# lyclyc52/Segment-Anything-NeRF

Measured on AMD Instinct MI355X. Metric: rays/sec (RGB+256-d SAM feat) at 512×512, 1/2/4/8 MI355X; PSNR vs ref, higher is better.
Workload: dtype fp32-equivalent: fp32 in the reference's op order for everything that decides a discrete result (near/far, bins, proposal grids + MLPs, compositing, sample_pdf); grid_mlp (32->64->64->16 per sample), the SAM head (163->256x5) and the mask head (143->256->256->K per sample) as f16x3: each fp32 produc

## Files before the change

segment-anything-nerf_amd/csrc/raymarch.hip:

```cpp
#include <algorithm>
#include <cmath>
#include <cstdlib>
#include <cstring>
#include <type_traits>

#include "f16x3.h"
#include "raymarch_device.h"
#include "samnerf_common.h"
#include "sh_device.h"
#include "wave_box.h"

using namespace samnerf;

namespace samnerf {
int sam_head_forward(const samnerf_model* m, const float* rows, uint32_t N, float* samvit,
                     float* packed, hipStream_t s, uint32_t ld = 256u, bool pack = true);
size_t sam_head_packed_floats();
int mask_head_forward(const samnerf_model* m, const GridDesc<16>& grid, const float* u_f, const float* w_f,
                      const float* geo_f, uint32_t N, float* out, RayTiles tiles, float* packed,
                      hipStream_t s);
size_t mask_head_packed_floats();
size_t mask_train_workspace_bytes(uint32_t N);
size_t mask_train_workspace_bytes(int mask_kind, uint32_t N);
int mask_train_forward(const samnerf_model* m, const GridDesc<16>& grid, const float* u_f, const float* w_f,
// ... 1491 lines not shown
}

struct SgridArgs {
    uint32_t N;
    RayTiles tiles;
    GridDesc<16> grid;
    const float* u_in;
    const float* w_in;
    float* rows;
    uint32_t* rows_tap;
    uint32_t tap_stride;
    unsigned long long* paths;
};


template <int T, int MODE>
__global__ void __launch_bounds__(256) k_sgrid(SgridArgs a) {
    constexpr int TQ = T / 4;
    __shared__ float part[3][8][64];
    const uint32_t lane = threadIdx.x & 63u, q = threadIdx.x >> 6;
    const uint32_t r = xcd_chunk(blockIdx.x, (a.N + 63u) / 64u) * 64u + lane;
    const uint32_t level = blockIdx.y;
    const bool live = r < a.N;
    const uint32_t N = a.N, rr = live ? r : N - 1;
    const LevelDesc lv = a.grid.lv[level];
    float acc[8];
#pragma unroll
    for (int c = 0; c < 8; ++c) acc[c] = 0.0f;
    const int k0 = (int)q * TQ;
    float ux = a.u_in[((size_t)k0 * 3 + 0) * N + rr];
    float uy = a.u_in[((size_t)k0 * 3 + 1) * N + rr];
    float uz = a.u_in[((size_t)k0 * 3 + 2) * N + rr];
    float w = a.w_in[(size_t)k0 * N + rr];
    for (int k = k0; k < k0 + TQ; ++k) {
        const int kn = k + 1 < k0 + TQ ? k + 1 : k;
        const float nx = a.u_in[((size_t)kn * 3 + 0) * N + rr];
        const float ny = a.u_in[((size_t)kn * 3 + 1) * N + rr];
        const float nz = a.u_in[((size_t)kn * 3 + 2) * N + rr];
        const float nw = a.w_in[(size_t)kn * N + rr];
        float f[8];
        if (__builtin_amdgcn_ballot_w64(w != 0.0f) == 0) {
        } else if constexpr (MODE == kLookRef) {
            lookup_level3_ref<8>(a.grid.emb, lv, ux, uy, uz, f);
#pragma unroll
            for (int c = 0; c < 8; ++c) acc[c] = acc[c] + w * f[c];
        } else {
            lookup_level3<8>(a.grid.emb, lv, ux, uy, uz, f);
            const f2v wv = {w, w};
#pragma unroll
            for (int c = 0; c < 8; c += 2) {
                const f2v s = f2v{acc[c], acc[c + 1]} + wv * f2v{f[c], f[c + 1]};
                acc[c] = s.x;
                acc[c + 1] = s.y;
            }
        }
        ux = nx;
        uy = ny;
        uz = nz;
        w = nw;
    }
    if (q > 0) {
#pragma unroll
        for (int c = 0; c < 8; ++c) part[q - 1][c][lane] = acc[c];
    }
    __syncthreads();
    if (q > 0 || !live) return;
#pragma unroll
    for (int c = 0; c < 8; ++c) acc[c] = ((acc[c] + part[0][c][lane]) + part[1][c][lane]) + part[2][c][lane];
    float4* dst = reinterpret_cast<float4*>(a.rows + (size_t)a.tiles(r) * kRow + level * 8u);
    dst[0] = make_float4(acc[0], acc[1], acc[2], acc[3]);
    dst[1] = make_float4(acc[4], acc[5], acc[6], acc[7]);
}

constexpr uint32_t kBoxSlots = 256;

#ifndef SAMNERF_DIAG_SGRID_WAVES
#define SAMNERF_DIAG_SGRID_WAVES 4
#endif
#ifndef SAMNERF_SGRID_UNI
#define SAMNERF_SGRID_UNI 1
#endif
constexpr bool SGRID_UNI = SAMNERF_SGRID_UNI;

template <int T, bool TAP = false>
__global__ void __launch_bounds__(256)
#if SAMNERF_DIAG_SGRID_WAVES
__attribute__((amdgpu_waves_per_eu(SAMNERF_DIAG_SGRID_WAVES, SAMNERF_DIAG_SGRID_WAVES)))
#endif
k_sgrid_box4(SgridArgs a) {
    constexpr int TQ = T / 4;
    __shared__ float4 smem[4][kBoxSlots * 2];
    const uint32_t lane = threadIdx.x & 63u, q = threadIdx.x >> 6;
    const uint32_t r = xcd_chunk(blockIdx.x, (a.N + 63u) / 64u) * 64u + lane;
    const uint32_t g = blockIdx.y;
    const bool live = r < a.N;
    const uint32_t N = a.N, rr = live ? r : N - 1;
    const LevelDesc L[4] = {a.grid.lv[4 * g], a.grid.lv[4 * g + 1], a.grid.lv[4 * g + 2],
                            a.grid.lv[4 * g + 3]};
    const uint32_t li = lane & 3u;
    const LevelDesc mine = {li == 0 ? L[0].off : li == 1 ? L[1].off : li == 2 ? L[2].off : L[3].off,
                            li == 0 ? L[0].size : li == 1 ? L[1].size : li == 2 ? L[2].size : L[3].size,
                            li == 0 ? L[0].res : li == 1 ? L[1].res : li == 2 ? L[2].res : L[3].res,
                            0u,
                            li == 0 ? L[0].fres : li == 1 ? L[1].fres : li == 2 ? L[2].fres : L[3].fres,
                            li == 0 ? L[0].ftop : li == 1 ? L[1].ftop : li == 2 ? L[2].ftop : L[3].ftop};
    float* slice = reinterpret_cast<float*>(smem[q]);
    const char* base = reinterpret_cast<const char*>(a.grid.emb);
    float acc[4][8];
#pragma unroll
    for (int l = 0; l < 4; ++l)
#pragma unroll
        for (int c = 0; c < 8; ++c) acc[l][c] = 0.0f;
    const int k0 = (int)q * TQ;
    const char* ub = reinterpret_cast<const char*>(a.u_in);
    const char* wb = reinterpret_cast<const char*>(a.w_in);
    const uint32_t N4 = N * 4u;
    auto ld = [](const char* b, uint32_t off) { return *reinterpret_cast<const float*>(b + off); };
    float ux = ld(ub, ((uint32_t)k0 * 3u + 0u) * N4 + rr * 4u);
    float uy = ld(ub, ((uint32_t)k0 * 3u + 1u) * N4 + rr * 4u);
    float uz = ld(ub, ((uint32_t)k0 * 3u + 2u) * N4 + rr * 4u);
    float w = ld(wb, (uint32_t)k0 * N4 + rr * 4u);
    for (int k = k0; k < k0 + TQ; ++k) {
        const uint32_t kn = (uint32_t)(k + 1 < k0 + TQ ? k + 1 : k);
        const float nx = ld(ub, (kn * 3u + 0u) * N4 + rr * 4u);
        const float ny = ld(ub, (kn * 3u + 1u) * N4 + rr * 4u);
        const float nz = ld(ub, (kn * 3u + 2u) * N4 + rr * 4u);
        const float nw = ld(wb, kn * N4 + rr * 4u);
#ifdef SAMNERF_DIAG_VARIANTS
        if (a.paths && lane == 0u && __builtin_amdgcn_ballot_w64(w != 0.0f) == 0) atomicAdd(a.paths + 3, 1ull);
#endif
        if (__builtin_amdgcn_ballot_w64(w != 0.0f) != 0) {
            const f2v wv = {w, w};
            auto add = [&](int l, const float* f) {
#pragma unroll
                for (int c = 0; c < 8; c += 2) {
                    const f2v s2 = f2v{acc[l][c], acc[l][c + 1]} + wv * f2v{f[c], f[c + 1]};
                    acc[l][c] = s2.x;
                    acc[l][c + 1] = s2.y;
                }
            };
            const URange ur = wave_urange(ux, uy, uz);
            const bool ordered = wave_positions_ordered(ux, uy, uz);
            uint32_t p0, p1, p2;
            pbox_lane(mine, ur, p0, p1, p2);
#pragma unroll
            for (int l = 0; l < 4; ++l) {
                const PBox b = pbox_read(p0, p1, p2, l);
                float f[8];
                uint32_t* rt = nullptr;
                if (TAP && live && r % a.tap_stride == 0u)
                    rt = a.rows_tap + ((size_t)(r / a.tap_stride) * T + k) * 128u + (4 * g + l) * 8;
#ifdef SAMNERF_DIAG_VARIANTS
                if (a.paths && lane == 0u) {
                    const int path = (SGRID_UNI && b.uni && ordered) ? 0 : b.slots <= kBoxSlots ? 1 : 2;
                    atomicAdd(a.paths + path, 1ull);
                    if (path == 1) {
                        atomicAdd(a.paths + 4, (unsigned long long)b.slots);
                        atomicAdd(a.paths + 5, (unsigned long long)(b.ex * b.ey * b.ez));
                    }
                }
#endif
                if (SGRID_UNI && b.uni && ordered) {
                    const uint32_t dx = b.ex - 1u, dy = b.ey - 1u, dz = b.ez - 1u;
                    uint32_t rows[8];
#pragma unroll
                    for (int c = 0; c < 8; ++c)
                        rows[c] = dense_or_hash_row(b.x0 + (c & 1) * dx, b.y0 + ((c >> 1) & 1) * dy,
                                                    b.z0 + (c >> 2) * dz, L[l]);
                    if (rt) {
#pragma unroll
                        for (int c = 0; c < 8; ++c) rt[c] = rows[c];
                    }
                    lookup_level3_uniform<8>(a.grid.emb, L[l], rows, ux, uy, uz, f);
                } else if (b.slots <= kBoxSlots) {
                    wave_lds_sync();
                    stage_pbox<8>(base, L[l], b, slice, lane);
                    wave_lds_sync();
                    if (ordered)
                        lookup_level3_pbox<8, false>(a.grid.emb, L[l], b, slice, ux, uy, uz, f, rt);
                    else
                        lookup_level3_pbox<8, true>(a.grid.emb, L[l], b, slice, ux, uy, uz, f, rt);
                } else {
                    if (rt) tap_direct_rows<8>(L[l], ux, uy, uz, rt);
                    lookup_level3<8>(a.grid.emb, L[l], ux, uy, uz, f);
                }
                add(l, f);
            }
        }
        ux = nx;
        uy = ny;
        uz = nz;
        w = nw;
    }
    __syncthreads();
    float* part = reinterpret_cast<float*>(smem);
    if (q > 0) {
#pragma unroll
        for (int l = 0; l < 4; ++l)
#pragma unroll
            for (int c = 0; c < 8; ++c) part[((q - 1) * 32 + l * 8 + c) * 64 + lane] = acc[l][c];
    }
    __syncthreads();
    if (q > 0 || !live) return;
    float* dst = a.rows + (size_t)a.tiles(r) * kRow + g * 32u;
#pragma unroll
    for (int l = 0; l < 4; ++l) {
        float v[8];
#pragma unroll
        for (int c = 0; c < 8; ++c) {
            const int i = l * 8 + c;
            v[c] = ((acc[l][c] + part[(0 * 32 + i) * 64 + lane]) + part[(1 * 32 + i) * 64 + lane]) +
                   part[(2 * 32 + i) * 64 + lane];
        }
        reinterpret_cast<float4*>(dst + l * 8)[0] = make_float4(v[0], v[1], v[2], v[3]);
        reinterpret_cast<float4*>(dst + l * 8)[1] = make_float4(v[4], v[5], v[6], v[7]);
    }
}

constexpr uint32_t kBwdBoxCells = 64;

struct DetAcc {
    unsigned long long* acc;
    const uint32_t* hdr;
    int log2n;
};

__device__ __forceinline__ bool sgrid_det_nonfinite(const DetAcc& d) { return d.hdr[1] != 0u; }

__device__ __forceinline__ int sgrid_det_shift(const DetAcc& d) {
    int e = 0;
    frexpf(__uint_as_float(d.hdr[0]), &e);
    return 61 - d.log2n - e;
}

template <int T, bool DET = false>
__global__ void __launch_bounds__(256)
k_sgrid_backward(uint32_t N, RayTiles tiles, GridDesc<16> g, const float* __restrict__ u_in,
                 const float* __restrict__ w_in, const float* __restrict__ grad, uint32_t gstride,
                 float* __restrict__ gemb, uint32_t max_cells, uint32_t run_res, DetAcc det = {}) {
    __shared__ float box[4][kBwdBoxCells * 8];
    __shared__ uint32_t list[4][kBwdBoxCells];
    const uint64_t t = (uint64_t)blockIdx.x * blockDim.x + threadIdx.x;
    const uint32_t r = (uint32_t)(t >> 3), ch = (uint32_t)(t & 7u), lane = threadIdx.x & 63u;
    const uint32_t wv = threadIdx.x >> 6;
    const uint32_t level = blockIdx.y;
    if (((t & ~(uint64_t)63) >> 3) >= N) return;
#ifdef SG_DIAG_MINLEVEL
    if (level < SG_DIAG_MINLEVEL) return;
#endif
    const bool live = r < N;
    const uint32_t rr = live ? r : N - 1;
    const LevelDesc d = g.lv[level];
    const float gv = live ? grad[(size_t)tiles(rr) * gstride + level * 8u + ch] : 0.0f;
    float* base = gemb + (size_t)d.off * 8u + ch;
    float* slice = box[wv];
    uint32_t* rows = list[wv];
    const uint32_t top = d.res - 1u;
    const int k0 = (int)(blockIdx.z * T / gridDim.z), k1 = (int)((blockIdx.z + 1) * T / gridDim.z);
    const bool run = !DET && max_cells == 0u && d.res <= run_res;
    const bool fixed = DET && !sgrid_det_nonfinite(det);
    const double dscale = fixed ? ldexp(1.0, sgrid_det_shift(det)) : 0.0;
    unsigned long long* const dbase = fixed ? det.acc + (size_t)d.off * 8u + ch : nullptr;
    uint32_t prow[8];
    float pval[8];
#pragma unroll
    for (int c = 0; c < 8; ++c) {
        prow[c] = 0xFFFFFFFFu;
        pval[c] = 0.0f;
    }
    for (int k = k0; k < k1; ++k) {
        const float ux = u_in[((size_t)k * 3 + 0) * N + rr];
        const float uy = u_in[((size_t)k * 3 + 1) * N + rr];
        const float uz = u_in[((size_t)k * 3 + 2) * N + rr];
        const float wk = w_in[(size_t)k * N + rr];
        if (__builtin_amdgcn_ballot_w64(wk != 0.0f) == 0) continue;
        const float wg = wk * gv;
        uint32_t cx, cy, cz;
        float fx, fy, fz;
        locate_axis(ux, d, cx, fx);
        locate_axis(uy, d, cy, fy);
        locate_axis(uz, d, cz, fz);
        const uint32_t nx = min(cx + 1u, top), ny = min(cy + 1u, top), nz = min(cz + 1u, top);
        const uint32_t x0 = (uint32_t)wave_imin((int)cx), x1 = (uint32_t)wave_imax((int)nx);
        const uint32_t y0 = (uint32_t)wave_imin((int)cy), y1 = (uint32_t)wave_imax((int)ny);
        const uint32_t z0 = (uint32_t)wave_imin((int)cz), z1 = (uint32_t)wave_imax((int)nz);
        const uint32_t ex = x1 - x0 + 1u, ey = y1 - y0 + 1u, ez = z1 - z0 + 1u;
        const uint32_t cells = ex * ey * ez;
        if (!DET && cells <= max_cells) {
            reinterpret_cast<float4*>(slice + lane * 8u)[0] = make_float4(0.0f, 0.0f, 0.0f, 0.0f);
            reinterpret_cast<float4*>(slice + lane * 8u)[1] = make_float4(0.0f, 0.0f, 0.0f, 0.0f);
            wave_lds_sync();
            const uint32_t X[2] = {cx - x0, nx - x0};
            const uint32_t Y[2] = {(cy - y0) * ex, (ny - y0) * ex};
            const uint32_t Z[2] = {(cz - z0) * ex * ey, (nz - z0) * ex * ey};
#pragma unroll
            for (int c = 0; c < 8; ++c) {
                const float wx = (c & 1) ? fx : 1.0f - fx;
                const float wy = (c & 2) ? fy : 1.0f - fy;
// ... 178 lines not shown
    z[r * 3] = a;
    z[r * 3 + 1] = b;
    z[r * 3 + 2] = c;
}

__global__ void __launch_bounds__(256)
k_sample_pdf(const float* __restrict__ bins, const float* __restrict__ weights, uint32_t N,
             uint32_t T0, uint32_t T, Lin u, float* __restrict__ out, int32_t* __restrict__ inds) {
    const uint32_t r = blockIdx.x * blockDim.x + threadIdx.x;
    if (r >= N) return;
    const float* w = weights + (size_t)r * T0;
    const float* b = bins + (size_t)r * (T0 + 1);
    const float wsum = torch_row_sum((int)T0, [&](int i) { return w[i] + 0.01f; });
    sample_pdf_walk(
        (int)T0, (int)T, u, wsum, [&](int i) { return w[i]; },
        [&](int i) { return b[i]; },
        [&](int j, float v, int ind) {
            out[(size_t)r * T + j] = v;
            if (inds) inds[(size_t)r * T + j] = ind;
        });
}

__global__ void __launch_bounds__(256)
k_composite(const float* __restrict__ rb, const float* __restrict__ sig, uint32_t N, uint32_t T,
            float* __restrict__ w) {
    const uint32_t r = blockIdx.x * blockDim.x + threadIdx.x;
    if (r >= N) return;
    double cum = 0.0;
    for (uint32_t k = 0; k < T; ++k) {
        const float ds = (rb[(size_t)r * (T + 1) + k + 1] - rb[(size_t)r * (T + 1) + k]) *
                         sig[(size_t)r * T + k];
        w[(size_t)r * T + k] = composite_step(ds, cum, k == T - 1);
    }
}

}



namespace {

struct Workspace {
    float* snf;
    float4* rec;
    float* bins1;
    float* bins2;
    float* wtmp;
    float* u_f;
    float* w_f;
    float* rows;
    float* packed;
    uint4* gpack;
    int* gexp;
    float* geo_f;
    float* mpacked;
    float* aeff;
    float* mlog;
    float* xsum;
    uint32_t* n1_list;
    uint32_t* n1_cnt;
    uint64_t* n1_mask;
    uint32_t* n1_base;
    double* n1_std;
    float* n1_stf;
    size_t bytes;
};

size_t align256(size_t b) { return (b + 255) & ~(size_t)255; }

int lookup_mode() {
    const char* v = diag_env("SAMNERF_LOOKUP");
    if (!v || !*v) return kLookAuto;
    if (!strcmp(v, "ref")) return kLookRef;
    if (!strcmp(v, "box")) return kLookBox4;
    if (!strcmp(v, "box4")) return kLookBox4;
    return kLookPacked;
}

thread_local hipEvent_t g_stage_events[8];
thread_local uint32_t g_n_stage_events = 0;
thread_local samnerf_taps g_taps = {};
thread_local uint32_t g_taps_n = 0;
thread_local bool g_taps_on = false;
thread_local uint32_t g_last_forms[4] = {};

void mark_stage(uint32_t i, hipStream_t s) {
    if (i < g_n_stage_events && g_stage_events[i]) (void)hipEventRecord(g_stage_events[i], s);
}

constexpr uint32_t kBox4MinRays = 32768;

uint32_t final_classes() {
    const char* v = diag_env("SAMNERF_FINAL_CLASSES");
    return (v && atoi(v) == 0) ? 0u : 1u;
}

int final_layout(const FinalArgs& fa) {
    const char* v = diag_env("SAMNERF_FINAL_LAY");
    if (v && atoi(v) == 0) return 0;
    for (int kb = 0; kb < 2; ++kb)
        if (fa.kdense[kb] != kLay1Dense[kb] || fa.khashed[kb] != kLay1Hashed[kb]) return 0;
    if (fa.hbit == 0u) return 0;
    return fa.gs.inv_b2 != 0.0f ? 1 : 0;
}

void set_hash_slots(FinalArgs& fa, const GridDesc<16>& g) {
    fa.hbit = fa.hm8 = 0u;
    uint32_t S = 0u;
    for (int kb = 0; kb < 2; ++kb)
        for (int q = 0; q < 4; ++q) {
            fa.hoff8[kb][q] = 0u;
            if (!((fa.khashed[kb] >> q) & 1u)) continue;
            const LevelDesc& a = g.lv[final_level(kb, 0, q)];
            const LevelDesc& b = g.lv[final_level(kb, 1, q)];
            if (!S) S = a.size;
            if (a.size != S || b.size != S || (S & (S - 1u)) || b.off != a.off + S || a.res > S || b.res > S ||
                (uint64_t)S * 8u > (1ull << 31))
                return;
            fa.hoff8[kb][q] = a.off * 8u;
        }
    if (!S) return;
    fa.hbit = S * 8u;
    fa.hm8 = (S - 1u) * 8u;
}

bool pack_weights(const samnerf_model* m) {
#ifdef SAMNERF_DIAG_VARIANTS
    return true;
#else
    return m->reuse_packed == 0;
#endif
}

bool box4_ok(const GridDesc<16>& g) {
    for (int l = 0; l < 16; ++l)
        if (g.lv[l].res > 1023u) return false;
    return true;
}

template <int T, bool FIRST>
void launch_prop_sigma(int look, uint32_t N, hipStream_t s, const PropArgs& pa) {
    const uint32_t nb = prop_sigma_blocks<T>(N);
    uint32_t kd = 0, kh = 0;
    for (int l = 0; l < 5; ++l) {
        kd |= (pa.grid.lv[l].flags & kHashed) ? 0u : 1u << l;
        kh |= (pa.grid.lv[l].flags & kHashed) ? 1u << l : 0u;
    }
    const char* pl = diag_env("SAMNERF_PROP_LAY");
    bool small_res = true;
    for (int l = 0; l < 5; ++l)
        if ((pa.grid.lv[l].flags & kHashed) && pa.grid.lv[l].res > pa.grid.lv[l].size) small_res = false;
    const bool lay = (look == kLookPacked || look == kLookAuto) && pa.gs.inv_b2 != 0.0f &&
                     !(pl && atoi(pl) == 0) && small_res && pa.rec;
    const bool lay_ok = lay && ((kd == 0x07u && kh == 0x18u) || (kd == 0x03u && kh == 0x1Cu));
    g_last_forms[T == 128 ? 0 : 1] = lay_ok ? kd | kh << 8 : 0u;
    if (lay && kd == 0x07u && kh == 0x18u) {
        k_prop_sigma<T, FIRST, kLookPacked, 0x07u, 0x18u><<<nb, 256, 0, s>>>(pa);
        return;
    }
    if (lay && kd == 0x03u && kh == 0x1Cu) {
        k_prop_sigma<T, FIRST, kLookPacked, 0x03u, 0x1Cu><<<nb, 256, 0, s>>>(pa);
        return;
    }
    if (look == kLookRef) k_prop_sigma<T, FIRST, kLookRef><<<nb, 256, 0, s>>>(pa);
    else if (look == kLookBox4 && box4_ok(pa.grid))
        k_prop_sigma<T, FIRST, kLookBox4><<<nb, 256, 0, s>>>(pa);
    else k_prop_sigma<T, FIRST, kLookPacked><<<nb, 256, 0, s>>>(pa);
}

struct EffArgs {
    const float* w[8];
    uint32_t K;
    int kind;
// ... 494 lines not shown
    }
    set_hash_slots(fa, gg);
    fa.G0 = m->grid_mlp[0];
    fa.G1 = m->grid_mlp[1];
    fa.G2 = m->grid_mlp[2];
    fa.V0 = m->view_mlp[0];
    fa.V1 = m->view_mlp[1];
    fa.V2 = m->view_mlp[2];
    fa.bins_in = bins2;
    fa.snf = w.snf;
    fa.u_out = w.u_f;
    fa.w_out = w.w_f;
    fa.image = image;
    fa.depth = depth;
    fa.wsum = weights_sum;
    fa.img_ld = ol.img_ld;
    fa.scal_ld = ol.scal_ld;
    if (!(m->t_thresh >= 0.0f && m->t_thresh < 1.0f))
        return fail(SAMNERF_EINVAL, "render_forward: t_thresh %g outside [0, 1)", (double)m->t_thresh);
    fa.exit_depth = m->t_thresh > 0.0f ? -logf(m->t_thresh) : INFINITY;
    if (tp.row_stride == 0 && (tp.rows2 || tp.srows))
        return fail(SAMNERF_EINVAL, "render: taps rows2 / srows need row_stride > 0");
    fa.sigma_tap = tp.sigma2;
    fa.rows_tap = tp.rows2;
    fa.tap_stride = tp.row_stride ? tp.row_stride : 1u;
    fa.i0 = 0;
    fa.i1 = 32;
    if (m->t_thresh > 0.0f) {
        fa.n1.list = w.n1_list;
        fa.n1.cnt = w.n1_cnt;
        fa.n1.mask = w.n1_mask;
        fa.n1.base = w.n1_base;
        fa.st_d = w.n1_std;
        fa.st_f = w.n1_stf;
    }
    int ad = 0;
    if (m->with_mask) {
        if (m->t_thresh > 0.0f)
            return fail(SAMNERF_EINVAL, "render_forward: the mask head and t_thresh do not combine");
        if (m->mask_kind < 0 || m->mask_kind > 2)
            return fail(SAMNERF_EINVAL, "render_forward: mask_kind %d", m->mask_kind);
        if (m->mask_out < 1 || m->mask_out > 32)
            return fail(SAMNERF_EINVAL, "render_forward: mask_out %u outside 1..32", m->mask_out);
        const int nl = m->mask_kind == 0 ? 3 : m->mask_kind == 1 ? 6 : 8;
        for (int i = 0; i < nl; ++i)
            if (!m->mask_w[i]) return fail(SAMNERF_EINVAL, "render_forward: null mask_mlp weight %d", i);
        if (m->mask_kind == 0) {
            fa.geo_out = w.geo_f;
        } else {
            if (m->mask_kind == 2 && !m->sum_after_mlp)
                return fail(SAMNERF_EINVAL, "render_forward: the adaptive 'rgb' head needs sum_after_mlp");
            EffArgs ea{};
            for (int i = 0; i < nl; ++i) ea.w[i] = m->mask_w[i];
            ea.K = m->mask_out;
            ea.kind = m->mask_kind;
            ea.aeff = w.aeff;
            k_mask_eff<<<1, 256, 0, s>>>(ea);
            fa.aeff = w.aeff;
            fa.mlog = w.mlog;
            fa.xsum = m->with_mask == 2 ? w.xsum : nullptr;
            fa.mask_out = m->mask_out;
            ad = m->mask_kind;
        }
    }
    const bool sam_rows = m->with_sam && (samvit || feature_rows);
    fa.rows = sam_rows || feature_rows ? rows : nullptr;
    mark_stage(2, s);
    const char* fs = diag_env("SAMNERF_FINAL_S");
    const bool n1_passes = m->t_thresh > 0.0f && n1_chunks() > 1;
    const int seg = fs ? atoi(fs) : (n1_passes || N >= 65536u ? 1 : N >= 32768u ? 2 : 4);
    fa.i1 = 32 / seg;
    if (m->sum_after_mlp && (m->t_thresh > 0.0f || sam_rows))
        return fail(SAMNERF_EINVAL, "render_forward: sum_after_mlp renders RGB (+ mask) only: no SAM "
                    "features (the reference's branch crashes, SURVEY 0.2) and no t_thresh");
    if (m->head_mode == 1) {
        launch_final<true>(seg, N, s, fa, m->sum_after_mlp != 0, ad);
    } else {
        fa.gpack = w.gpack;
        fa.gexp = w.gexp;
        if (pack_weights(m)) k_pack_grid_mlp<<<1, 256, 0, s>>>(fa, w.gpack, w.gexp);
        launch_final<false>(seg, N, s, fa, m->sum_after_mlp != 0, ad);
    }

    if (sam_rows) {
        SgridArgs sa{};
        sa.N = N;
        sa.tiles = tiles;
        sa.grid = gs;
        sa.u_in = w.u_f;
        sa.w_in = w.w_f;
        sa.rows = rows;
        sa.rows_tap = tp.srows;
        sa.tap_stride = tp.row_stride ? tp.row_stride : 1u;
        {
            const char* pp = diag_env("SAMNERF_SGRID_PATHS");
            sa.paths = pp ? reinterpret_cast<unsigned long long*>(strtoull(pp, nullptr, 16)) : nullptr;
        }
        mark_stage(3, s);
        const dim3 sg(xcd_blocks(div_up(N, 64)), 16);
        const dim3 sb(xcd_blocks(div_up(N, 64)), 4);
        if (look == kLookRef) {
            k_sgrid<32, kLookRef><<<sg, 256, 0, s>>>(sa);
        } else if ((look == kLookBox4 || (look == kLookAuto && N >= kBox4MinRays)) && box4_ok(gs) &&
                   (uint64_t)N * 384u < (1ull << 32)) {
            if (sa.rows_tap) k_sgrid_box4<32, true><<<sb, 256, 0, s>>>(sa);
            else k_sgrid_box4<32><<<sb, 256, 0, s>>>(sa);
        } else {
            k_sgrid<32, kLookPacked><<<sg, 256, 0, s>>>(sa);
        }
        if ((rc = check_launch("render"))) return rc;
        mark_stage(4, s);
        if (samvit) rc = sam_head_forward(m, rows, N, samvit, w.packed, s, ol.sv_ld, pack_weights(m));
        mark_stage(5, s);
        if (rc == SAMNERF_OK) rc = copy_final_taps(tp, w, N, s);
        return rc;
    }
    mark_stage(3, s);
    mark_stage(4, s);
    mark_stage(5, s);
    if ((rc = check_launch("render"))) return rc;
    return copy_final_taps(tp, w, N, s);
}

}

extern "C" {

int samnerf_render_forward(const samnerf_model* m, const float* rays_o, const float* rays_d,
                           uint32_t N, const float* cam_near_far, uint32_t n_cnf, float bg_color,
                           float* image, float* depth, float* weights_sum, float* samvit,
                           float* feature_rows, void* workspace, size_t workspace_bytes,
                           samnerf_stream_t stream) {
    if (!m) return fail(SAMNERF_EINVAL, "render: null pointer");
    if (N == 0) return SAMNERF_OK;
    if (!rays_o || !rays_d || !image || !depth || !weights_sum)
        return fail(SAMNERF_EINVAL, "render: null pointer");
    const OutLayout ol{image, depth, weights_sum, samvit, 3u, 1u, 256u};
    return render_impl(m, rays_o, rays_d, N, cam_near_far, n_cnf, bg_color, ol, feature_rows, workspace,
                       workspace_bytes, stream);
}

int samnerf_render_forward_tile(const samnerf_model* m, const float* rays_o, const float* rays_d,
                                uint32_t N, const float* cam_near_far, uint32_t n_cnf, float bg_color,
                                float* tile, uint32_t ld, int feats, float* feature_rows, void* workspace,
                                size_t workspace_bytes, samnerf_stream_t stream) {
    if (!m) return fail(SAMNERF_EINVAL, "render_tile: null pointer");
    if (N == 0) return SAMNERF_OK;
    if (!rays_o || !rays_d || !tile) return fail(SAMNERF_EINVAL, "render_tile: null pointer");
    const bool sv = feats && m->with_sam;
    if (ld < (sv ? 261u : 5u))
        return fail(SAMNERF_EINVAL, "render_tile: row of %u floats cannot hold the outputs (needs %u)", ld,
                    sv ? 261u : 5u);
    const OutLayout ol{tile, tile + 3, tile + 4, sv ? tile + 5 : nullptr, ld, ld, ld};
    return render_impl(m, rays_o, rays_d, N, cam_near_far, n_cnf, bg_color, ol, feature_rows, workspace,
                       workspace_bytes, stream);
}

int samnerf_set_stage_events(void* const* events, uint32_t n) {
    if (n > 8) return fail(SAMNERF_EINVAL, "set_stage_events: at most 8 events");
    g_n_stage_events = events ? n : 0u;
    for (uint32_t i = 0; i < g_n_stage_events; ++i)
        g_stage_events[i] = reinterpret_cast<hipEvent_t>(events[i]);
    return SAMNERF_OK;
}

int samnerf_last_forms(uint32_t* out, uint32_t n) {
    for (uint32_t i = 0; out && i < n && i < 4; ++i) out[i] = g_last_forms[i];
    return 4;
}

int samnerf_clock_stamp(uint64_t* out, samnerf_stream_t stream) {
    if (!out) return fail(SAMNERF_EINVAL, "clock_stamp: null pointer");
    k_clock_stamp<<<256, 64, 0, reinterpret_cast<hipStream_t>(stream)>>>(
        reinterpret_cast<unsigned long long*>(out));
    return check_launch("clock_stamp");
}

int samnerf_set_taps(const samnerf_taps* taps, uint32_t N) {
    g_taps_on = taps != nullptr;
    g_taps = taps ? *taps : samnerf_taps{};
    g_taps_n = taps ? N : 0u;
    return SAMNERF_OK;
}

int samnerf_mask_forward(const samnerf_model* m, uint32_t N, float* logits, const void* workspace,
                         size_t workspace_bytes, samnerf_stream_t stream) {
    if (!m) return fail(SAMNERF_EINVAL, "mask_forward: null model");
    if (!m->with_mask) return fail(SAMNERF_EINVAL, "mask_forward: model has no mask head (with_mask = 0)");
    if (N == 0) return SAMNERF_OK;
    if (!logits || !workspace) return fail(SAMNERF_EINVAL, "mask_forward: null pointer");
    if (m->mask_out < 1 || m->mask_out > 32)
        return fail(SAMNERF_EINVAL, "mask_forward: mask_out %u outside 1..32", m->mask_out);
    if (m->num_steps[2] != 32) return fail(SAMNERF_EINVAL, "mask_forward: fused path is built for 32 final samples");
    Workspace w = carve(m, N, const_cast<void*>(workspace));
    if (workspace_bytes < w.bytes)
        return fail(SAMNERF_EWORKSPACE, "mask_forward: workspace needs %zu bytes, got %zu", w.bytes,
                    workspace_bytes);
    if (m->mask_kind != 0) {
        if (hipMemcpyAsync(logits, w.mlog, sizeof(float) * m->mask_out * (size_t)N, hipMemcpyDeviceToDevice,
                           reinterpret_cast<hipStream_t>(stream)) != hipSuccess)
            return fail(SAMNERF_ELAUNCH, "mask_forward: copy failed");
        return SAMNERF_OK;
    }
    for (int i = 0; i < 3; ++i)
        if (!m->mask_w[i]) return fail(SAMNERF_EINVAL, "mask_forward: null mask_mlp weight");
    GridDesc<16> gm;
    int rc = make_grid_desc(m->m_grid, 8, 16, gm, "m_grid");
    if (rc) return rc;
    const RayTiles tiles = make_ray_tiles(N, m->view_width);
    return mask_head_forward(m, gm, w.u_f, w.w_f, w.geo_f, N, logits, tiles, w.mpacked,
                             reinterpret_cast<hipStream_t>(stream));
}

size_t samnerf_mask_train_workspace_size(uint32_t N) { return mask_train_workspace_bytes(N); }

size_t samnerf_mask_train_workspace_size_model(const samnerf_model* m, uint32_t N) {
    if (!m || !m->with_mask || m->mask_kind < 0 || m->mask_kind > 2) return mask_train_workspace_bytes(N);
    return mask_train_workspace_bytes(m->mask_kind, N);
}

static int mask_train_inputs(const samnerf_model* m, uint32_t N, const void* render_ws, size_t render_bytes,
                             Workspace& w, GridDesc<16>& gm, const char* what) {
    if (!m) return fail(SAMNERF_EINVAL, "%s: null model", what);
    if (!m->with_mask || m->mask_kind < 0 || m->mask_kind > 2)
        return fail(SAMNERF_EINVAL, "%s: model has no fused mask head (with_mask = 1, mask_kind 0-2)", what);
    if (m->mask_out < 1 || m->mask_out > 32)
        return fail(SAMNERF_EINVAL, "%s: mask_out %u outside 1..32", what, m->mask_out);
    if (m->num_steps[2] != 32) return fail(SAMNERF_EINVAL, "%s: fused path is built for 32 final samples", what);
    if (!render_ws) return fail(SAMNERF_EINVAL, "%s: null render workspace", what);
    w = carve(m, N, const_cast<void*>(render_ws));
    if (render_bytes < w.bytes)
        return fail(SAMNERF_EWORKSPACE, "%s: render workspace needs %zu bytes, got %zu", what, w.bytes,
                    render_bytes);
    if (m->mask_kind != 0 && m->with_mask != 2)
        return fail(SAMNERF_EINVAL, "%s: the adaptive heads train on a render with with_mask = 2 (it keeps "
                    "the per-ray input sums)", what);
    return m->mask_kind == 0 ? make_grid_desc(m->m_grid, 8, 16, gm, "m_grid") : SAMNERF_OK;
}

int samnerf_mask_train_forward(const samnerf_model* m, uint32_t N, float* logits, const void* render_ws,
                               size_t render_bytes, void* workspace, size_t workspace_bytes,
                               samnerf_stream_t stream) {
    Workspace w;
    GridDesc<16> gm;
    int rc = mask_train_inputs(m, N, render_ws, render_bytes, w, gm, "mask_train_forward");
    if (rc) return rc;
    if (N == 0) return SAMNERF_OK;
    if (!logits || !workspace) return fail(SAMNERF_EINVAL, "mask_train_forward: null pointer");
    if (m->mask_kind != 0)
        return adaptive_train_forward(m, w.xsum, N, logits, workspace, workspace_bytes,
                                      reinterpret_cast<hipStream_t>(stream));
// ... 103 lines not shown
```

segment-anything-nerf_amd/csrc/wave_box.h:

```cpp
#pragma once

#include <hip/hip_runtime.h>
#include <limits.h>
#include <stdint.h>

#include "samnerf_common.h"

namespace samnerf {

template <int CTRL>
__device__ __forceinline__ float dpp_f(float v) {
    return __int_as_float(__builtin_amdgcn_update_dpp(0, __float_as_int(v), CTRL, 0xf, 0xf, false));
}

__device__ __forceinline__ float wave_fmin(float v) {
    v = fminf(v, dpp_f<0xB1>(v));
    v = fminf(v, dpp_f<0x4E>(v));
    v = fminf(v, dpp_f<0x141>(v));
    v = fminf(v, dpp_f<0x140>(v));
    const int b = __float_as_int(v);
    const float r0 = __int_as_float(__builtin_amdgcn_readlane(b, 0));
    const float r1 = __int_as_float(__builtin_amdgcn_readlane(b, 16));
    const float r2 = __int_as_float(__builtin_amdgcn_readlane(b, 32));
    const float r3 = __int_as_float(__builtin_amdgcn_readlane(b, 48));
// ... 27 lines not shown
    v = min(v, dpp_i<0x4E>(v));
    v = min(v, dpp_i<0x141>(v));
    v = min(v, dpp_i<0x140>(v));
    const int r0 = __builtin_amdgcn_readlane(v, 0), r1 = __builtin_amdgcn_readlane(v, 16);
    const int r2 = __builtin_amdgcn_readlane(v, 32), r3 = __builtin_amdgcn_readlane(v, 48);
    return min(min(r0, r1), min(r2, r3));
}

__device__ __forceinline__ int wave_imax(int v) {
    v = max(v, dpp_i<0xB1>(v));
    v = max(v, dpp_i<0x4E>(v));
    v = max(v, dpp_i<0x141>(v));
    v = max(v, dpp_i<0x140>(v));
    const int r0 = __builtin_amdgcn_readlane(v, 0), r1 = __builtin_amdgcn_readlane(v, 16);
    const int r2 = __builtin_amdgcn_readlane(v, 32), r3 = __builtin_amdgcn_readlane(v, 48);
    return max(max(r0, r1), max(r2, r3));
}

__device__ __forceinline__ URange wave_urange(float ux, float uy, float uz) {
    const float u[3] = {ux, uy, uz};
    int lo[3], hi[3];
#pragma unroll
    for (int c = 0; c < 3; ++c) {
        const int b = __float_as_int(u[c]);
        const bool nan = u[c] != u[c];
        lo[c] = nan ? INT_MAX : b;
        hi[c] = nan ? INT_MIN : b;
    }
#define SAMNERF_URANGE_STEP(EXPR_LO, EXPR_HI)                                   \
    _Pragma("unroll") for (int c = 0; c < 3; ++c) {                             \
        lo[c] = min(lo[c], EXPR_LO);                                            \
        hi[c] = max(hi[c], EXPR_HI);                                            \
    }
    SAMNERF_URANGE_STEP(dpp_i<0xB1>(lo[c]), dpp_i<0xB1>(hi[c]))
    SAMNERF_URANGE_STEP(dpp_i<0x4E>(lo[c]), dpp_i<0x4E>(hi[c]))
    SAMNERF_URANGE_STEP(dpp_i<0x141>(lo[c]), dpp_i<0x141>(hi[c]))
    SAMNERF_URANGE_STEP(dpp_i<0x140>(lo[c]), dpp_i<0x140>(hi[c]))
    SAMNERF_URANGE_STEP(__builtin_amdgcn_update_dpp(INT_MAX, lo[c], 0x142, 0xa, 0xf, false),
                        __builtin_amdgcn_update_dpp(INT_MIN, hi[c], 0x142, 0xa, 0xf, false))
    SAMNERF_URANGE_STEP(__builtin_amdgcn_update_dpp(INT_MAX, lo[c], 0x143, 0xc, 0xf, false),
                        __builtin_amdgcn_update_dpp(INT_MIN, hi[c], 0x143, 0xc, 0xf, false))
#undef SAMNERF_URANGE_STEP
    URange r;
#pragma unroll
    for (int c = 0; c < 3; ++c) {
        r.lo[c] = __int_as_float(__builtin_amdgcn_readlane(lo[c], 63));
        r.hi[c] = __int_as_float(__builtin_amdgcn_readlane(hi[c], 63));
    }
    return r;
}

__device__ __forceinline__ uint32_t cell_of(float u, const LevelDesc& d) {
    float p = __builtin_fmaf(u, d.fres, -0.5f);
    p = clamp_med3(p, d.ftop);
    return (uint32_t)p;
}

}

namespace samnerf {


__device__ __forceinline__ uint32_t log2_ceil(uint32_t v) { return v <= 1u ? 0u : 32u - __clz(v - 1u); }

struct PBox {
    uint32_t x0, y0, z0, ex, ey, ez, lx, ly, slots;
    uint32_t uni;
};

__device__ __forceinline__ void pbox_lane(const LevelDesc& d, const URange& u, uint32_t& p0,
                                          uint32_t& p1, uint32_t& p2) {
    const uint32_t top = d.res - 1u;
    const uint32_t x0 = cell_of(u.lo[0], d), y0 = cell_of(u.lo[1], d), z0 = cell_of(u.lo[2], d);
    const uint32_t hx = cell_of(u.hi[0], d), hy = cell_of(u.hi[1], d), hz = cell_of(u.hi[2], d);
    const uint32_t x1 = min(hx + 1u, top);
    const uint32_t y1 = min(hy + 1u, top);
    const uint32_t z1 = min(hz + 1u, top);
    const uint32_t ex = x1 - x0 + 1u, ey = y1 - y0 + 1u, ez = z1 - z0 + 1u;
    p0 = x0 | (y0 << 10) | (z0 << 20);
    p1 = ex | (ey << 10) | (ez << 20);
    p2 = log2_ceil(ex) | (log2_ceil(ey) << 8) | ((hx == x0 && hy == y0 && hz == z0) ? 1u << 16 : 0u);
}

__device__ __forceinline__ PBox pbox_read(uint32_t p0, uint32_t p1, uint32_t p2, int lane) {
    const uint32_t a = (uint32_t)__builtin_amdgcn_readlane((int)p0, lane);
    const uint32_t b = (uint32_t)__builtin_amdgcn_readlane((int)p1, lane);
    const uint32_t c = (uint32_t)__builtin_amdgcn_readlane((int)p2, lane);
    PBox r;
    r.x0 = a & 1023u;
    r.y0 = (a >> 10) & 1023u;
    r.z0 = a >> 20;
    r.ex = b & 1023u;
    r.ey = (b >> 10) & 1023u;
    r.ez = b >> 20;
    r.lx = c & 255u;
    r.ly = (c >> 8) & 255u;
    r.uni = c >> 16;
    r.slots = r.ez << (r.lx + r.ly);
    return r;
}

template <int C>
__device__ __forceinline__ void stage_pbox(const char* __restrict__ base, const LevelDesc& d,
                                           const PBox& b, float* slice, uint32_t lane) {
    const uint32_t xm = (1u << b.lx) - 1u, ym = (1u << b.ly) - 1u;
    for (uint32_t j = lane; j < b.slots; j += 64u) {
        const uint32_t bx = j & xm, t = j >> b.lx, by = t & ym, bz = t >> b.ly;
        if (bx < b.ex && by < b.ey) {
            const uint32_t row = dense_or_hash_row(b.x0 + bx, b.y0 + by, b.z0 + bz, d);
            float e[C];
            load_row_b<C>(base, (d.off + row) * (uint32_t)(C * 4), e);
            if constexpr (C == 2) {
                *reinterpret_cast<float2*>(slice + j * 2) = make_float2(e[0], e[1]);
            } else {
#pragma unroll
                for (int i = 0; i < C; i += 4)
                    *reinterpret_cast<float4*>(slice + j * C + i) = make_float4(e[i], e[i + 1], e[i + 2], e[i + 3]);
            }
        }
    }
}

__device__ __forceinline__ void wave_lds_sync() {
    __builtin_amdgcn_fence(__ATOMIC_ACQ_REL, "wavefront");
    __builtin_amdgcn_wave_barrier();
}

__device__ __forceinline__ bool wave_positions_ordered(float ux, float uy, float uz) {
    return __builtin_amdgcn_ballot_w64(ux != ux || uy != uy || uz != uz) == 0;
}

template <int C>
__device__ __forceinline__ void tap_direct_rows(const LevelDesc& d, float ux, float uy, float uz,
                                                uint32_t* tap) {
    uint32_t off[8];
    float w[8];
    corner_rows<C>(d, ux, uy, uz, off, w);
#pragma unroll
    for (int c = 0; c < 8; ++c) tap[c] = off[c] / (uint32_t)(C * 4) - d.off;
}

template <int C>
__device__ __forceinline__ void lookup_level3_uniform(const float* __restrict__ emb, const LevelDesc& d,
                                                      const uint32_t* row, float ux, float uy, float uz,
                                                      float* acc) {
    static_assert(C == 8, "uniform-cell lookup: C = 8 rows (32 B)");
    uint32_t cx, cy, cz;
    float fx, fy, fz;
    locate_axis(ux, d, cx, fx);
    locate_axis(uy, d, cy, fy);
    locate_axis(uz, d, cz, fz);
    f2v wc[4];
    corner_weights_pk(fx, fy, fz, wc);
    f2v a[C / 2];
#pragma unroll
    for (int i = 0; i < C / 2; ++i) a[i] = f2v{0.0f, 0.0f};
#pragma unroll
    for (int c = 0; c < 8; ++c) {
        const float4* p = reinterpret_cast<const float4*>(emb + (size_t)(d.off + row[c]) * C);
        const float4 v0 = p[0], v1 = p[1];
        const float w = corner_w(wc, c);
        const f2v wv = {w, w};
        a[0] = __builtin_elementwise_fma(wv, f2v{v0.x, v0.y}, a[0]);
        a[1] = __builtin_elementwise_fma(wv, f2v{v0.z, v0.w}, a[1]);
        a[2] = __builtin_elementwise_fma(wv, f2v{v1.x, v1.y}, a[2]);
        a[3] = __builtin_elementwise_fma(wv, f2v{v1.z, v1.w}, a[3]);
    }
#pragma unroll
    for (int i = 0; i < C / 2; ++i) {
        acc[2 * i] = a[i].x;
        acc[2 * i + 1] = a[i].y;
    }
}

template <int C, bool CHECK = true>
__device__ __forceinline__ void lookup_level3_pbox(const float* __restrict__ emb, const LevelDesc& d,
                                                   const PBox& b, const float* slice, float ux,
                                                   float uy, float uz, float* acc,
                                                   uint32_t* tap = nullptr) {
    uint32_t cx, cy, cz;
    float fx, fy, fz;
    locate_axis(ux, d, cx, fx);
    locate_axis(uy, d, cy, fy);
    locate_axis(uz, d, cz, fz);
    const uint32_t top = d.res - 1u;
    const uint32_t nx = min(cx + 1u, top), ny = min(cy + 1u, top), nz = min(cz + 1u, top);
    const uint32_t lx0 = cx - b.x0, lx1 = nx - b.x0;
    const uint32_t ly0 = cy - b.y0, ly1 = ny - b.y0;
    const uint32_t lz0 = cz - b.z0, lz1 = nz - b.z0;
    if constexpr (CHECK) {
        const bool inside = lx0 < b.ex && lx1 < b.ex && ly0 < b.ey && ly1 < b.ey && lz0 < b.ez && lz1 < b.ez;
        if (!inside) {
            if (tap) tap_direct_rows<C>(d, ux, uy, uz, tap);
            lookup_level3<C>(emb, d, ux, uy, uz, acc);
            return;
        }
    }
    constexpr uint32_t RB = C * 4u;
    const uint32_t lxy = b.lx + b.ly;
    const uint32_t o0 = (lx0 + (ly0 << b.lx) + (lz0 << lxy)) * RB;
    const uint32_t DX = (lx1 - lx0) * RB, DY = ((ly1 - ly0) << b.lx) * RB, DZ = ((lz1 - lz0) << lxy) * RB;
    uint32_t off[8];
    off[0] = o0;
    off[1] = o0 + DX;
    off[2] = o0 + DY;
    off[3] = off[2] + DX;
    off[4] = o0 + DZ;
    off[5] = off[4] + DX;
    off[6] = off[4] + DY;
    off[7] = off[6] + DX;
    if (tap) {
        const uint32_t xm = (1u << b.lx) - 1u, ym = (1u << b.ly) - 1u;
#pragma unroll
        for (int c = 0; c < 8; ++c) {
            const uint32_t j = off[c] / RB;
            tap[c] = dense_or_hash_row(b.x0 + (j & xm), b.y0 + ((j >> b.lx) & ym), b.z0 + (j >> lxy), d);
        }
    }
    f2v wc[4];
    corner_weights_pk(fx, fy, fz, wc);
    const char* sb = reinterpret_cast<const char*>(slice);
    f2v a[C / 2];
#pragma unroll
    for (int i = 0; i < C / 2; ++i) a[i] = f2v{0.0f, 0.0f};
#pragma unroll
    for (int c = 0; c < 8; ++c) {
        const float w = corner_w(wc, c);
        const f2v wv = {w, w};
        if constexpr (C == 2) {
            const float2 v = *reinterpret_cast<const float2*>(sb + off[c]);
            a[0] = __builtin_elementwise_fma(wv, f2v{v.x, v.y}, a[0]);
        } else {
#pragma unroll
            for (int i = 0; i < C; i += 4) {
                const float4 v = *reinterpret_cast<const float4*>(sb + off[c] + i * 4);
                a[i / 2] = __builtin_elementwise_fma(wv, f2v{v.x, v.y}, a[i / 2]);
                a[i / 2 + 1] = __builtin_elementwise_fma(wv, f2v{v.z, v.w}, a[i / 2 + 1]);
            }
        }
    }
#pragma unroll
    for (int i = 0; i < C / 2; ++i) {
        acc[2 * i] = a[i].x;
// ... 6 lines not shown
```

Before: 95.81 million.

## Add merged all-level sgrid box kernel with precomputed box plans and scalar loads

Adds k_sgrid_box4_merged, which has one block walk all four level groups. Per-sample box descriptors are precomputed once into LDS plans, samples with zero weight are skipped wave-wide, and sample positions are reused across groups instead of being reloaded by four separate y-blocks. The merged kernel is reachable only through an env var or a compile-time ray threshold that defaults to never. The change that is always on is in the uniform-cell lookup: the wave-uniform row offset goes through readfirstlane and a constant-address-space pointer, so the corner embeddings can be fetched with scalar loads. The per-level dispatch is also factored into a shared helper.

```diff
diff --git a/segment-anything-nerf_amd/csrc/raymarch.hip b/segment-anything-nerf_amd/csrc/raymarch.hip
--- a/segment-anything-nerf_amd/csrc/raymarch.hip
+++ b/segment-anything-nerf_amd/csrc/raymarch.hip
@@ -1597,6 +1597,45 @@
 #endif
 constexpr bool SGRID_UNI = SAMNERF_SGRID_UNI;
 
+__device__ __forceinline__ void sgrid_box_level(const SgridArgs& a, const LevelDesc& L, const PBox& b,
+                                                bool ordered, float* slice, uint32_t lane, float ux,
+                                                float uy, float uz, float* f, uint32_t* rt) {
+#ifdef SAMNERF_DIAG_VARIANTS
+    if (a.paths && lane == 0u) {
+        const int path = (SGRID_UNI && b.uni && ordered) ? 0 : b.slots <= kBoxSlots ? 1 : 2;
+        atomicAdd(a.paths + path, 1ull);
+        if (path == 1) {
+            atomicAdd(a.paths + 4, (unsigned long long)b.slots);
+            atomicAdd(a.paths + 5, (unsigned long long)(b.ex * b.ey * b.ez));
+        }
+    }
+#endif
+    if (SGRID_UNI && b.uni && ordered) {
+        const uint32_t dx = b.ex - 1u, dy = b.ey - 1u, dz = b.ez - 1u;
+        uint32_t rows[8];
+#pragma unroll
+        for (int c = 0; c < 8; ++c)
+            rows[c] = dense_or_hash_row(b.x0 + (c & 1) * dx, b.y0 + ((c >> 1) & 1) * dy,
+                                        b.z0 + (c >> 2) * dz, L);
+        if (rt) {
+#pragma unroll
+            for (int c = 0; c < 8; ++c) rt[c] = rows[c];
+        }
+        lookup_level3_uniform<8>(a.grid.emb, L, rows, ux, uy, uz, f);
+    } else if (b.slots <= kBoxSlots) {
+        wave_lds_sync();
+        stage_pbox<8>(reinterpret_cast<const char*>(a.grid.emb), L, b, slice, lane);
+        wave_lds_sync();
+        if (ordered)
+            lookup_level3_pbox<8, false>(a.grid.emb, L, b, slice, ux, uy, uz, f, rt);
+        else
+            lookup_level3_pbox<8, true>(a.grid.emb, L, b, slice, ux, uy, uz, f, rt);
+    } else {
+        if (rt) tap_direct_rows<8>(L, ux, uy, uz, rt);
+        lookup_level3<8>(a.grid.emb, L, ux, uy, uz, f);
+    }
+}
+
 template <int T, bool TAP = false>
 __global__ void __launch_bounds__(256)
 #if SAMNERF_DIAG_SGRID_WAVES
@@ -1620,7 +1659,6 @@
                             li == 0 ? L[0].fres : li == 1 ? L[1].fres : li == 2 ? L[2].fres : L[3].fres,
                             li == 0 ? L[0].ftop : li == 1 ? L[1].ftop : li == 2 ? L[2].ftop : L[3].ftop};
     float* slice = reinterpret_cast<float*>(smem[q]);
-    const char* base = reinterpret_cast<const char*>(a.grid.emb);
     float acc[4][8];
 #pragma unroll
     for (int l = 0; l < 4; ++l)
@@ -1665,40 +1703,7 @@
                 uint32_t* rt = nullptr;
                 if (TAP && live && r % a.tap_stride == 0u)
                     rt = a.rows_tap + ((size_t)(r / a.tap_stride) * T + k) * 128u + (4 * g + l) * 8;
-#ifdef SAMNERF_DIAG_VARIANTS
-                if (a.paths && lane == 0u) {
-                    const int path = (SGRID_UNI && b.uni && ordered) ? 0 : b.slots <= kBoxSlots ? 1 : 2;
-                    atomicAdd(a.paths + path, 1ull);
-                    if (path == 1) {
-                        atomicAdd(a.paths + 4, (unsigned long long)b.slots);
-                        atomicAdd(a.paths + 5, (unsigned long long)(b.ex * b.ey * b.ez));
-                    }
-                }
-#endif
-                if (SGRID_UNI && b.uni && ordered) {
-                    const uint32_t dx = b.ex - 1u, dy = b.ey - 1u, dz = b.ez - 1u;
-                    uint32_t rows[8];
-#pragma unroll
-                    for (int c = 0; c < 8; ++c)
-                        rows[c] = dense_or_hash_row(b.x0 + (c & 1) * dx, b.y0 + ((c >> 1) & 1) * dy,
-                                                    b.z0 + (c >> 2) * dz, L[l]);
-                    if (rt) {
-#pragma unroll
-                        for (int c = 0; c < 8; ++c) rt[c] = rows[c];
-                    }
-                    lookup_level3_uniform<8>(a.grid.emb, L[l], rows, ux, uy, uz, f);
-                } else if (b.slots <= kBoxSlots) {
-                    wave_lds_sync();
-                    stage_pbox<8>(base, L[l], b, slice, lane);
-                    wave_lds_sync();
-                    if (ordered)
-                        lookup_level3_pbox<8, false>(a.grid.emb, L[l], b, slice, ux, uy, uz, f, rt);
-                    else
-                        lookup_level3_pbox<8, true>(a.grid.emb, L[l], b, slice, ux, uy, uz, f, rt);
-                } else {
-                    if (rt) tap_direct_rows<8>(L[l], ux, uy, uz, rt);
-                    lookup_level3<8>(a.grid.emb, L[l], ux, uy, uz, f);
-                }
+                sgrid_box_level(a, L[l], b, ordered, slice, lane, ux, uy, uz, f, rt);
                 add(l, f);
             }
         }
@@ -1729,6 +1734,149 @@
         }
         reinterpret_cast<float4*>(dst + l * 8)[0] = make_float4(v[0], v[1], v[2], v[3]);
         reinterpret_cast<float4*>(dst + l * 8)[1] = make_float4(v[4], v[5], v[6], v[7]);
+    }
+}
+
+constexpr uint32_t kPlanWords = 49;
+
+template <int T>
+__global__ void __launch_bounds__(256)
+#if SAMNERF_DIAG_SGRID_WAVES
+__attribute__((amdgpu_waves_per_eu(SAMNERF_DIAG_SGRID_WAVES, SAMNERF_DIAG_SGRID_WAVES)))
+#endif
+k_sgrid_box4_merged(SgridArgs a) {
+    constexpr int TQ = T / 4;
+    __shared__ float4 smem[4][kBoxSlots * 2];
+    __shared__ uint32_t plans[4][TQ * kPlanWords];
+    static_assert(4 * (sizeof(smem) + sizeof(plans)) <= 160u * 1024u, "k_sgrid_box4_merged: LDS");
+    static_assert(sizeof(float) * 32 * 64 == sizeof(smem[0]), "the quarter hand-off fills one slice");
+    const uint32_t lane = threadIdx.x & 63u, q = (uint32_t)__builtin_amdgcn_readfirstlane(threadIdx.x >> 6);
+    const uint32_t r0 = xcd_chunk(blockIdx.x, (a.N + 63u) / 64u) * 64u, r = r0 + lane;
+    if (r0 >= a.N) return;
+    const bool live = r < a.N;
+    const uint32_t N = a.N, rr = live ? r : N - 1;
+    float* slice = reinterpret_cast<float*>(smem[q]);
+    uint32_t* plan = plans[q];
+    const int k0 = (int)q * TQ;
+    const char* ub = reinterpret_cast<const char*>(a.u_in);
+    const char* wb = reinterpret_cast<const char*>(a.w_in);
+    const uint32_t N4 = N * 4u;
+    auto ld = [](const char* b, uint32_t off) { return *reinterpret_cast<const float*>(b + off); };
+    {
+        const uint32_t li = lane & 15u;
+        LevelDesc mine = {0u, 0u, a.grid.lv[0].res, 0u, a.grid.lv[0].fres, a.grid.lv[0].ftop};
+#pragma unroll
+        for (int l = 1; l < 16; ++l) {
+            mine.res = li == (uint32_t)l ? a.grid.lv[l].res : mine.res;
+            mine.fres = li == (uint32_t)l ? a.grid.lv[l].fres : mine.fres;
+            mine.ftop = li == (uint32_t)l ? a.grid.lv[l].ftop : mine.ftop;
+        }
+        uint32_t* mp = plan + (li >> 2) * 12u + (li & 3u);
+#pragma unroll 2
+        for (int s = 0; s < TQ; ++s) {
+            const uint32_t k = (uint32_t)(k0 + s);
+            const float ux = ld(ub, (k * 3u + 0u) * N4 + rr * 4u);
+            const float uy = ld(ub, (k * 3u + 1u) * N4 + rr * 4u);
+            const float uz = ld(ub, (k * 3u + 2u) * N4 + rr * 4u);
+            const float w = ld(wb, k * N4 + rr * 4u);
+            const bool any = __builtin_amdgcn_ballot_w64(w != 0.0f) != 0;
+            const bool ordered = wave_positions_ordered(ux, uy, uz);
+            if (lane == 16u) plan[s * kPlanWords + 48u] = (any ? 1u : 0u) | (ordered ? 2u : 0u);
+            if (any) {
+                const URange ur = wave_urange(ux, uy, uz);
+                uint32_t p0, p1, p2;
+                pbox_lane(mine, ur, p0, p1, p2);
+                if (lane < 16u) {
+                    mp[s * kPlanWords] = p0;
+                    mp[s * kPlanWords + 4u] = p1;
+                    mp[s * kPlanWords + 8u] = p2;
+                }
+            }
+        }
+    }
+    wave_lds_sync();
+    const float* part = reinterpret_cast<const float*>(smem);
+    const uint32_t drow = a.tiles(rr);
+    LevelDesc L[4] = {a.grid.lv[0], a.grid.lv[1], a.grid.lv[2], a.grid.lv[3]};
+    float acc[4][8];
+#pragma unroll
+    for (int l = 0; l < 4; ++l)
+#pragma unroll
+        for (int c = 0; c < 8; ++c) acc[l][c] = 0.0f;
+    float ux = ld(ub, ((uint32_t)k0 * 3u + 0u) * N4 + rr * 4u);
+    float uy = ld(ub, ((uint32_t)k0 * 3u + 1u) * N4 + rr * 4u);
+    float uz = ld(ub, ((uint32_t)k0 * 3u + 2u) * N4 + rr * 4u);
+    float w = ld(wb, (uint32_t)k0 * N4 + rr * 4u);
+    uint32_t pl = plan[lane < 12u ? lane : 48u];
+#pragma unroll 1
+    for (uint32_t it = 0; it < 4u * TQ; ++it) {
+        const uint32_t g = it / TQ, s = it % TQ;
+        const bool last = s + 1u == (uint32_t)TQ;
+        const uint32_t sn = last ? 0u : s + 1u, gn = last && g < 3u ? g + 1u : g;
+        const uint32_t kn = (uint32_t)k0 + sn;
+        const float nx = ld(ub, (kn * 3u + 0u) * N4 + rr * 4u);
+        const float ny = ld(ub, (kn * 3u + 1u) * N4 + rr * 4u);
+        const float nz = ld(ub, (kn * 3u + 2u) * N4 + rr * 4u);
+        const float nw = ld(wb, kn * N4 + rr * 4u);
+        const uint32_t npl = plan[sn * kPlanWords + (lane < 12u ? gn * 12u + lane : 48u)];
+        const uint32_t flags = (uint32_t)__builtin_amdgcn_readlane((int)pl, 12);
+#ifdef SAMNERF_DIAG_VARIANTS
+        if (a.paths && lane == 0u && !(flags & 1u)) atomicAdd(a.paths + 3, 1ull);
+#endif
+        if (flags & 1u) {
+            const bool ordered = (flags & 2u) != 0u;
+            const f2v wv = {w, w};
+#pragma unroll
+            for (int l = 0; l < 4; ++l) {
+                const PBox b = pbox_unpack((uint32_t)__builtin_amdgcn_readlane((int)pl, l),
+                                           (uint32_t)__builtin_amdgcn_readlane((int)pl, 4 + l),
+                                           (uint32_t)__builtin_amdgcn_readlane((int)pl, 8 + l));
+                float f[8];
+                sgrid_box_level(a, L[l], b, ordered, slice, lane, ux, uy, uz, f, nullptr);
+#pragma unroll
+                for (int c = 0; c < 8; c += 2) {
+                    const f2v s2 = f2v{acc[l][c], acc[l][c + 1]} + wv * f2v{f[c], f[c + 1]};
+                    acc[l][c] = s2.x;
+                    acc[l][c + 1] = s2.y;
+                }
+            }
+        }
+        ux = nx;
+        uy = ny;
+        uz = nz;
+        w = nw;
+        pl = npl;
+        if (!last) continue;
+        wave_lds_sync();
+        if (q > 0) {
+#pragma unroll
+            for (int l = 0; l < 4; ++l)
+#pragma unroll
+                for (int c = 0; c < 8; ++c) slice[(l * 8 + c) * 64 + lane] = acc[l][c];
+        }
+        __syncthreads();
+        if (q == 0 && live) {
+            float* dst = a.rows + (size_t)drow * kRow + g * 32u;
+#pragma unroll
+            for (int l = 0; l < 4; ++l) {
+                float v[8];
+#pragma unroll
+                for (int c = 0; c < 8; ++c) {
+                    const int i = l * 8 + c;
+                    v[c] = ((acc[l][c] + part[(1 * 32 + i) * 64 + lane]) + part[(2 * 32 + i) * 64 + lane]) +
+                           part[(3 * 32 + i) * 64 + lane];
+                }
+                reinterpret_cast<float4*>(dst + l * 8)[0] = make_float4(v[0], v[1], v[2], v[3]);
+                reinterpret_cast<float4*>(dst + l * 8)[1] = make_float4(v[4], v[5], v[6], v[7]);
+            }
+        }
+        __syncthreads();
+#pragma unroll
+        for (int l = 0; l < 4; ++l) {
+            L[l] = a.grid.lv[4u * gn + l];
+#pragma unroll
+            for (int c = 0; c < 8; ++c) acc[l][c] = 0.0f;
+        }
     }
 }
 
@@ -2073,13 +2221,17 @@
 thread_local samnerf_taps g_taps = {};
 thread_local uint32_t g_taps_n = 0;
 thread_local bool g_taps_on = false;
-thread_local uint32_t g_last_forms[4] = {};
+thread_local uint32_t g_last_forms[5] = {};
 
 void mark_stage(uint32_t i, hipStream_t s) {
     if (i < g_n_stage_events && g_stage_events[i]) (void)hipEventRecord(g_stage_events[i], s);
 }
 
 constexpr uint32_t kBox4MinRays = 32768;
+#ifndef SAMNERF_BOX4_MERGED_MIN_RAYS
+#define SAMNERF_BOX4_MERGED_MIN_RAYS 0xFFFFFFFFu
+#endif
+constexpr uint32_t kBox4MergedMinRays = SAMNERF_BOX4_MERGED_MIN_RAYS;
 
 uint32_t final_classes() {
     const char* v = diag_env("SAMNERF_FINAL_CLASSES");
@@ -2740,6 +2892,7 @@
         launch_final<false>(seg, N, s, fa, m->sum_after_mlp != 0, ad);
     }
 
+    g_last_forms[4] = 0u;
     if (sam_rows) {
         SgridArgs sa{};
         sa.N = N;
@@ -2757,12 +2910,23 @@
         mark_stage(3, s);
         const dim3 sg(xcd_blocks(div_up(N, 64)), 16);
         const dim3 sb(xcd_blocks(div_up(N, 64)), 4);
+        const dim3 sm(xcd_blocks(div_up(N, 64)), 1);
+        const char* sf = diag_env("SAMNERF_SGRID_FORM");
+        const int form = !sf || !*sf ? 0 : !strcmp(sf, "merged") ? 2 : 1;
         if (look == kLookRef) {
             k_sgrid<32, kLookRef><<<sg, 256, 0, s>>>(sa);
-        } else if ((look == kLookBox4 || (look == kLookAuto && N >= kBox4MinRays)) && box4_ok(gs) &&
+        } else if ((look == kLookBox4 || (look == kLookAuto && (form || N >= kBox4MinRays))) && box4_ok(gs) &&
                    (uint64_t)N * 384u < (1ull << 32)) {
-            if (sa.rows_tap) k_sgrid_box4<32, true><<<sb, 256, 0, s>>>(sa);
-            else k_sgrid_box4<32><<<sb, 256, 0, s>>>(sa);
+            if (sa.rows_tap) {
+                k_sgrid_box4<32, true><<<sb, 256, 0, s>>>(sa);
+                g_last_forms[4] = 1u;
+            } else if (form ? form == 2 : N >= kBox4MergedMinRays) {
+                k_sgrid_box4_merged<32><<<sm, 256, 0, s>>>(sa);
+                g_last_forms[4] = 2u;
+            } else {
+                k_sgrid_box4<32><<<sb, 256, 0, s>>>(sa);
+                g_last_forms[4] = 1u;
+            }
         } else {
             k_sgrid<32, kLookPacked><<<sg, 256, 0, s>>>(sa);
         }
@@ -2823,8 +2987,8 @@
 }
 
 int samnerf_last_forms(uint32_t* out, uint32_t n) {
-    for (uint32_t i = 0; out && i < n && i < 4; ++i) out[i] = g_last_forms[i];
-    return 4;
+    for (uint32_t i = 0; out && i < n && i < 5; ++i) out[i] = g_last_forms[i];
+    return 5;
 }
 
 int samnerf_clock_stamp(uint64_t* out, samnerf_stream_t stream) {
diff --git a/segment-anything-nerf_amd/csrc/wave_box.h b/segment-anything-nerf_amd/csrc/wave_box.h
--- a/segment-anything-nerf_amd/csrc/wave_box.h
+++ b/segment-anything-nerf_amd/csrc/wave_box.h
@@ -133,10 +133,7 @@
     p2 = log2_ceil(ex) | (log2_ceil(ey) << 8) | ((hx == x0 && hy == y0 && hz == z0) ? 1u << 16 : 0u);
 }
 
-__device__ __forceinline__ PBox pbox_read(uint32_t p0, uint32_t p1, uint32_t p2, int lane) {
-    const uint32_t a = (uint32_t)__builtin_amdgcn_readlane((int)p0, lane);
-    const uint32_t b = (uint32_t)__builtin_amdgcn_readlane((int)p1, lane);
-    const uint32_t c = (uint32_t)__builtin_amdgcn_readlane((int)p2, lane);
+__device__ __forceinline__ PBox pbox_unpack(uint32_t a, uint32_t b, uint32_t c) {
     PBox r;
     r.x0 = a & 1023u;
     r.y0 = (a >> 10) & 1023u;
@@ -149,6 +146,12 @@
     r.uni = c >> 16;
     r.slots = r.ez << (r.lx + r.ly);
     return r;
+}
+
+__device__ __forceinline__ PBox pbox_read(uint32_t p0, uint32_t p1, uint32_t p2, int lane) {
+    return pbox_unpack((uint32_t)__builtin_amdgcn_readlane((int)p0, lane),
+                       (uint32_t)__builtin_amdgcn_readlane((int)p1, lane),
+                       (uint32_t)__builtin_amdgcn_readlane((int)p2, lane));
 }
 
 template <int C>
@@ -206,10 +209,13 @@
     f2v a[C / 2];
 #pragma unroll
     for (int i = 0; i < C / 2; ++i) a[i] = f2v{0.0f, 0.0f};
+    typedef float f4c __attribute__((ext_vector_type(4)));
 #pragma unroll
     for (int c = 0; c < 8; ++c) {
-        const float4* p = reinterpret_cast<const float4*>(emb + (size_t)(d.off + row[c]) * C);
-        const float4 v0 = p[0], v1 = p[1];
+        const uint32_t ro = (uint32_t)__builtin_amdgcn_readfirstlane((int)(d.off + row[c]));
+        const __attribute__((address_space(4))) f4c* p =
+            (const __attribute__((address_space(4))) f4c*)(emb + (size_t)ro * C);
+        const f4c v0 = p[0], v1 = p[1];
         const float w = corner_w(wc, c);
         const f2v wv = {w, w};
         a[0] = __builtin_elementwise_fma(wv, f2v{v0.x, v0.y}, a[0]);
```

Result: no change. 95.02 million (-0.8%).
